# zellerlab/GECCO

Measured on AMD Instinct MI355X. Metric: genes/sec CRF decode (windowed fwd-bwd marginals + Viterbi), higher is better.
Workload: dtype f64

## Files before the change

gecco_amd/csrc/crf_vd_short.hpp:

```cpp
#pragma once

#include "crf_device.hpp"
#include "crf_scan.hpp"

namespace gecco {
namespace {

constexpr int kT = 256;
constexpr int kGPL = kSeqGenesPerLane;
constexpr int kBlockGenes = kT * kGPL;
static_assert(kBlockGenes == kSeqBlockGenes, "host tables assume this block size");

__device__ __forceinline__ double vd_max(double a, double b) {
    double r;
    asm("v_max_f64 %0, %1, %2" : "=v"(r) : "v"(a), "v"(b));
    return r;
}
__device__ __forceinline__ double vd_min(double a, double b) {
    double r;
    asm("v_min_f64 %0, %1, %2" : "=v"(r) : "v"(a), "v"(b));
    return r;
}
__device__ __forceinline__ double vd_min_abs(double a, double b) {
    double r;
    asm("v_min_f64 %0, |%1|, |%2|" : "=v"(r) : "v"(a), "v"(b));
    return r;
}
__device__ __forceinline__ double vd_max_s(double a, double bound) {
    double r;
    asm("v_max_f64 %0, %1, %2" : "=v"(r) : "v"(a), "s"(bound));
    return r;
}
__device__ __forceinline__ double vd_min_s(double a, double bound) {
    double r;
    asm("v_min_f64 %0, %1, %2" : "=v"(r) : "v"(a), "s"(bound));
    return r;
}
__device__ __forceinline__ void vd_shift_in_gt(uint32_t &acc, double x, double bound) {
    asm("v_cmp_lt_f64 vcc, %2, %1\n\tv_addc_co_u32 %0, vcc, %0, %0, vcc" : "+v"(acc) : "v"(x), "s"(bound) : "vcc");
}
struct COp {
    static __device__ __forceinline__ CE identity() { return CE{0.0, -__builtin_huge_val(), __builtin_huge_val()}; }
    static __device__ __forceinline__ CE combine(const CE &a, const CE &b) {
        return CE{a.a + b.a, vd_min(vd_max(a.L + b.a, b.L), b.H), vd_min(vd_max(a.H + b.a, b.L), b.H)};
    }
    static __device__ __forceinline__ void combine_into(CE &t, CE &v) {
        asm volatile(
            "v_add_f64 %[tl], %[tl], %[a]\n\t"
            "v_add_f64 %[th], %[th], %[a]\n\t"
            "v_add_f64 %[a], %[ta], %[a]\n\t"
            "v_max_f64 %[tl], %[tl], %[L]\n\t"
            "v_max_f64 %[th], %[th], %[L]\n\t"
            "v_min_f64 %[L], %[tl], %[H]\n\t"
            "v_min_f64 %[H], %[th], %[H]"
            : [a] "+v"(v.a), [L] "+v"(v.L), [H] "+v"(v.H), [tl] "+v"(t.L), [th] "+v"(t.H)
            : [ta] "v"(t.a));
    }
};

__device__ __forceinline__ double vd_bound(const SeqArgs &A, double nnz, double n) { return nnz * A.v_wmax2 + (n + 2.0) * A.v_tmax; }
constexpr double kVdEps = 2.220446049250313e-16;
__device__ __forceinline__ double vd_margin(double r, double ulpM) { return (4.0 * r + 4.0) * ulpM; }

constexpr int kFixChunk = 1024;
struct FixStage {
    double2 st[kFixChunk];
    uint32_t bpw[kFixChunk / 16];
};
__device__ __forceinline__ void exact_states(const SeqArgs &A, int g0, int m, FixStage &fx, int first_lane) {
    const int nl = kT - first_lane, me = int(threadIdx.x) - first_lane;
    if (me < 0) return;
    for (int base = me; base < m; base += 4 * nl) {
        int lo[4], hi[4];
        double s0[4], s1[4];
        int longest = 0;
#pragma unroll
        for (int u = 0; u < 4; ++u) {
            const int i = base + u * nl;
            lo[u] = hi[u] = 0;
            if (i < m) {
                lo[u] = A.csr_gene_ptr[g0 + i];
                hi[u] = A.csr_gene_ptr[g0 + i + 1];
            }
            s0[u] = s1[u] = 0.0;
        }
#pragma unroll
        for (int u = 0; u < 4; ++u) longest = max(longest, hi[u] - lo[u]);
        for (int k = 0; k < longest; ++k) {
            int a[4];
#pragma unroll
            for (int u = 0; u < 4; ++u) a[u] = lo[u] + k < hi[u] ? A.csr_attr_id[lo[u] + k] : -1;
            double2 w[4];
#pragma unroll
            for (int u = 0; u < 4; ++u) w[u] = unsigned(a[u]) < unsigned(A.csr_n_attrs) ? A.csr_wtab01[a[u]] : make_double2(0.0, 0.0);
#pragma unroll
            for (int u = 0; u < 4; ++u) {
                s0[u] += w[u].x;
                s1[u] += w[u].y;
            }
        }
#pragma unroll
        for (int u = 0; u < 4; ++u) {
            const int i = base + u * nl;
            if (i < m) fx.st[i] = make_double2(s0[u], s1[u]);
        }
    }
}
__device__ __forceinline__ void exact_walk(const SeqArgs &A, FixStage &fx, int m, bool first, double &d0, double &d1) {
    int i = 0;
    if (first) {
        d0 = fx.st[0].x;
        d1 = fx.st[0].y;
        i = 1;
    }
    auto step = [&](const double2 s) {
        const double a0 = d0 + A.t00, b0 = d1 + A.t10;
        const double a1 = d0 + A.t01, b1 = d1 + A.t11;
        d0 = fmax(a0, b0) + s.x;
        d1 = fmax(a1, b1) + s.y;
    };
    for (; i < m && (i & 7); ++i) {
        step(fx.st[i]);
        fx.st[i] = make_double2(d0, d1);
    }
    for (; i + 8 <= m; i += 8) {
        double2 sv[8];
#pragma unroll
        for (int u = 0; u < 8; ++u) sv[u] = fx.st[i + u];
#pragma unroll
        for (int u = 0; u < 8; ++u) {
            step(sv[u]);
            fx.st[i + u] = make_double2(d0, d1);
        }
    }
    for (; i < m; ++i) {
        step(fx.st[i]);
        fx.st[i] = make_double2(d0, d1);
    }
}
__device__ __forceinline__ void exact_backpointers(const SeqArgs &A, FixStage &fx, int m, bool first, double e0, double e1) {
    for (int w = threadIdx.x; 16 * w < m; w += kT) {
        uint32_t word = 0;
        for (int i = max(16 * w, first ? 1 : 0); i < min(16 * w + 16, m); ++i) {
            const double p0 = i ? fx.st[i - 1].x : e0, p1 = i ? fx.st[i - 1].y : e1;
            const uint32_t arg0 = (p0 + A.t00) < (p1 + A.t10) ? 1u : 0u, arg1 = (p0 + A.t01) < (p1 + A.t11) ? 1u : 0u;
            word |= (arg0 | (arg1 << 1)) << (2 * (i & 15));
        }
        fx.bpw[w] = word;
    }
}
__device__ __forceinline__ uint32_t *exact_bp_words(const SeqArgs &A, int gs) { return reinterpret_cast<uint32_t *>(A.alpha) + size_t(gs); }
__device__ __forceinline__ uint32_t *exact_end_labels(const SeqArgs &A, int gs) {
    return reinterpret_cast<uint32_t *>(A.alpha) + size_t(A.n_genes) + size_t(gs);
}
__device__ __forceinline__ void exact_backtrack(const SeqArgs &A, int gs, int ge, double d0, double d1) {
    const int n = ge - gs, nw = (n + 15) / 16;
    uint32_t *bpc = exact_bp_words(A, gs), *endl = exact_end_labels(A, gs);
    auto word_map = [&](uint32_t bits, int w, uint32_t y) {
        const int hi = min(16 * w + 15, n - 1), lo = max(16 * w, 1);
        for (int t = hi; t >= lo; --t) y = (bits >> (2 * (t & 15) + y)) & 1u;
        return y;
    };
    for (int w = threadIdx.x; w < nw; w += kT) {
        const uint32_t bits = bpc[w];
        endl[w] = word_map(bits, w, 0) | (word_map(bits, w, 1) << 1);
    }
    __syncthreads();
    if (threadIdx.x == 0) {
        uint32_t y = d0 < d1 ? 1u : 0u;
        for (int w = nw - 1; w >= 0; --w) {
            const uint32_t mp = endl[w];
            endl[w] = y;
            y = (mp >> y) & 1u;
        }
    }
    __syncthreads();
    for (int w = threadIdx.x; w < nw; w += kT) {
        const uint32_t bits = bpc[w];
        uint32_t y = endl[w];
        const int hi = min(16 * w + 15, n - 1), lo = 16 * w;
        for (int t = hi; t >= lo; --t) {
            A.y[gs + t] = int8_t(y);
            if (t >= 1) y = (bits >> (2 * (t & 15) + y)) & 1u;
        }
    }
    __syncthreads();
}

__device__ __forceinline__ void exact_delta_contig(const SeqArgs &A, int gs, int ge, FixStage &fx) {
    uint32_t *bpc = exact_bp_words(A, gs);
    double d0 = 0.0, d1 = 0.0;
    for (int cb = gs; cb < ge; cb += kFixChunk) {
        const int m = min(kFixChunk, ge - cb);
        const double e0 = d0, e1 = d1;
        exact_states(A, cb, m, fx, 0);
        __syncthreads();
        if (threadIdx.x == 0) exact_walk(A, fx, m, cb == gs, d0, d1);
        __syncthreads();
        d0 = fx.st[m - 1].x;
        d1 = fx.st[m - 1].y;
        exact_backpointers(A, fx, m, cb == gs, e0, e1);
        __syncthreads();
        for (int i = threadIdx.x; i < (m + 15) / 16; i += kT) bpc[(cb - gs) / 16 + i] = fx.bpw[i];
        __syncthreads();
    }
    exact_backtrack(A, gs, ge, d0, d1);
}

constexpr double kVdPad = 1e30;

struct VdShortSmem {
    double st[kT * (kGPL + 1)];
    uint32_t mark[kBlockGenes / 32];
    int c_end;
    CE tot[kT / 64];
    uint32_t mtot[kT / 64];
    double pv[kT / 64];
    uint32_t pbad[kT / 64];
    uint32_t vote[kT / 64];
};
static_assert(sizeof(VdShortSmem) <= 20480, "eight workgroups per CU");
__device__ __forceinline__ void load_short(const double *__restrict__ v, int g0, int n, VdShortSmem &stg, double (&x)[kGPL]) {
    const int base = int(threadIdx.x) * kGPL;
    const double *vp = v + g0;
    double *row = stg.st + threadIdx.x * (kGPL + 1);
    const int wave_end = (__builtin_amdgcn_readfirstlane(int(threadIdx.x >> 6)) + 1) * 64 * kGPL;
    if (wave_end <= n) {
#pragma unroll
        for (int k = 0; k < kGPL; ++k) x[k] = vp[base + k];
#pragma unroll
        for (int k = 0; k < kGPL; ++k) row[k] = x[k];
        return;
    }
#pragma unroll
    for (int k = 0; k < kGPL; ++k) x[k] = vp[max(min(base + k, n - 1), 0)];
#pragma unroll
    for (int k = 0; k < kGPL; ++k) {
        x[k] = base + k < n ? x[k] : kVdPad;
        row[k] = x[k];
    }
}

__device__ __forceinline__ uint32_t wave_or_u32(uint32_t v) {
    v |= uint32_t(__builtin_amdgcn_update_dpp(0, int(v), 0x111, 0xF, 0xF, true));
    v |= uint32_t(__builtin_amdgcn_update_dpp(0, int(v), 0x112, 0xF, 0xF, true));
    v |= uint32_t(__builtin_amdgcn_update_dpp(0, int(v), 0x114, 0xF, 0xF, true));
    v |= uint32_t(__builtin_amdgcn_update_dpp(0, int(v), 0x118, 0xF, 0xF, true));
    v |= uint32_t(__builtin_amdgcn_update_dpp(0, int(v), 0x142, 0xA, 0xF, true));
    v |= uint32_t(__builtin_amdgcn_update_dpp(0, int(v), 0x143, 0xC, 0xF, true));
    return uint32_t(__builtin_amdgcn_readlane(int(v), 63));
}

constexpr int kVdRun = 6;
__device__ __forceinline__ void vd_apply(const CE &P, double in, double &v) {
    asm volatile("v_add_f64 %0, %1, %2\n\tv_max_f64 %0, %0, %3\n\tv_min_f64 %0, %0, %4" : "+v"(v) : "v"(in), "v"(P.a), "v"(P.L), "v"(P.H));
}
__device__ __forceinline__ void vd_propagate(const CE &P, double &v, uint64_t &known) {
    for (int it = 0; it < kVdRun; ++it) {
        const uint64_t todo = (known << 1) & ~known;
        if (!todo) break;
        const double in = dpp_f64_z<0x138>(v);
        if (__builtin_amdgcn_inverse_ballot_w64(todo)) vd_apply(P, in, v);
        known |= todo;
    }
}

__device__ __forceinline__ void vd_short_block(const SeqArgs &A, const int blk, VdShortSmem &stg) {
    CE *lds = stg.tot;
    uint32_t *ldsm = stg.mtot;
    const int slot = threadIdx.x;
    const int g0 = __builtin_amdgcn_readfirstlane(A.cblk[blk]), n = __builtin_amdgcn_readfirstlane(A.cblk[blk + 1]) - g0;
    const uint32_t bits = A.lane_bits[blk * kT + slot];
    const uint32_t first = bits & 0xffu, last = bits >> 8;
    const uint32_t wave_bits = wave_or_u32(bits);
    double x[kGPL];
    load_short(A.dstate, g0, n, stg, x);
    const int cnt = min(kGPL, n - slot * kGPL);
    const double *row = stg.st + slot * (kGPL + 1);
    CE P = COp::identity();
#pragma unroll
    for (int k = 0; k < kGPL; ++k) {
        const double dvk = x[k];
        const bool fst = (first >> k) & 1u;
        const double c = A.v_k + dvk;
        const double l2 = vd_min_s(vd_max_s(P.L, A.v_lo), A.v_hi) + c, h2 = vd_min_s(vd_max_s(P.H, A.v_lo), A.v_hi) + c;
        P.a += c;
        P.L = l2;
        P.H = h2;
        if ((wave_bits >> k) & 1u) {
            asm volatile("" ::: "memory");
            P.L = fst ? dvk : l2;
            P.H = fst ? dvk : h2;
        }
    }
    double Din;
    {
        const int wave = __builtin_amdgcn_readfirstlane(int(threadIdx.x >> 6));
        double v = P.L;
        uint64_t known = __builtin_amdgcn_ballot_w64(P.L == P.H);
        vd_propagate(P, v, known);
        const bool wave_bad = (known | (known - 1)) != ~uint64_t(0) || !(known & (wave ? (uint64_t(2) << kVdRun) - 1 : uint64_t(1)));
        if ((threadIdx.x & 63) == 63) stg.pv[wave] = v;
        block_or_post(wave_bad, stg.pbad);
        __syncthreads();
        if (block_or_read(stg.pbad)) {
            const CE M = block_scan_exclusive<COp, false, CE, kScanThreads, true, true>(P, lds, static_cast<CE *>(nullptr));
            Din = M.L;
        } else {
            const double carry = stg.pv[wave ? wave - 1 : 0];
            if (!(known & 1u)) {
                if ((threadIdx.x & 63) == 0) vd_apply(P, carry, v);
                known |= 1u;
                vd_propagate(P, v, known);
            }
            Din = dpp_f64<0x138, 0xF>(carry, v);
        }
    }
    double ulpM = 0.0, margin = 1e-6 * fmax(1.0, fmax(fabs(A.v_lo), fabs(A.v_hi)));
    if (A.csr_gene_ptr) {
        ulpM = vd_bound(A, double(A.csr_gene_ptr[g0 + n] - A.csr_gene_ptr[g0]), double(n)) * kVdEps;
        margin = vd_margin(double(n), ulpM);
    }
    ulpM = __hiloint2double(__builtin_amdgcn_readfirstlane(__double2hiint(ulpM)), __builtin_amdgcn_readfirstlane(__double2loint(ulpM)));
    margin = __hiloint2double(__builtin_amdgcn_readfirstlane(__double2hiint(margin)), __builtin_amdgcn_readfirstlane(__double2loint(margin)));
    uint32_t maps = 0, lane_map;
    bool sensitive = false;
    {
        double Dq = Din, nearest = __builtin_huge_val();
#pragma unroll
        for (int k = 0; k < kGPL; ++k) {
            const double dvk = row[k];
            const double stepped = vd_min_s(vd_max_s(Dq, A.v_lo), A.v_hi) + (A.v_k + dvk);
            Dq = stepped;
            if ((wave_bits >> k) & 1u) {
                asm volatile("" ::: "memory");
                Dq = ((first >> k) & 1u) ? dvk : stepped;
            }
            vd_shift_in_gt(maps, Dq, A.v_lo);
            vd_shift_in_gt(maps, Dq, A.v_hi);
            double dist = vd_min_abs(Dq - A.v_hi, Dq - A.v_lo);
            if ((wave_bits >> (8 + k)) & 1u) {
                asm volatile("" ::: "memory");
                const bool lst = (last >> k) & 1u;
                maps = lst ? ((maps & ~3u) | (Dq > 0.0 ? 3u : 0u)) : maps;
                dist = lst ? fabs(Dq) : dist;
            }
            nearest = vd_min(nearest, dist);
        }
        sensitive = nearest <= margin;
    }
    auto label_map = [&]() {
        uint32_t y0 = 0u, y1 = 1u;
#pragma unroll
        for (int k = kGPL - 1; k >= 0; --k) {
            y0 = __builtin_amdgcn_ubfe(maps, uint32_t(2 * (kGPL - 1 - k)) | y0, 1u);
            y1 = __builtin_amdgcn_ubfe(maps, uint32_t(2 * (kGPL - 1 - k)) | y1, 1u);
        }
        return y0 | (y1 << 1);
    };
    const bool lane_sensitive = sensitive && A.v_exact;
    int vote = lane_sensitive ? 1 : 0;
    uint32_t mtotal;
    lane_map = label_map();
    uint32_t lab = block_scan_exclusive_back<MapOp>(lane_map, ldsm, &mtotal, &vote, stg.vote) & 1u;
    const bool wg_sensitive = vote != 0;
    if (wg_sensitive) {
        double Dq = Din;
        uint64_t sat = 0;
#pragma unroll
        for (int k = 0; k < kGPL; ++k) {
            if (k < cnt) {
                const double dvk = row[k];
            Dq = ((first >> k) & 1u) ? dvk : fmin(fmax(Dq, A.v_lo), A.v_hi) + (A.v_k + dvk);
                const uint64_t c = Dq >= A.v_hi + margin ? 1u : (Dq <= A.v_lo - margin ? 2u : 0u);
                sat |= c << (8 * k);
            }
        }
        *reinterpret_cast<uint64_t *>(&stg.st[slot * (kGPL + 1) + kGPL]) = sat;
        __syncthreads();
    } else {
        sensitive = false;
    }
    bool lane_flagged = false;
    if (sensitive && cnt > 0) {
        double D = 0.0;
        int r = 0;
        auto certain = [&](double x) { return x >= A.v_hi + margin || x <= A.v_lo - margin; };
        if (!(first & 1u)) {
            const int t0 = slot * kGPL;
            int p = t0 - 1;
            auto dval = [&](int t) { return stg.st[(t / kGPL) * (kGPL + 1) + t % kGPL]; };
            for (;; --p) {
                if (A.flags[g0 + p] & 1u) {
                    D = dval(p);
                    r = 0;
                    break;
                }
                const uint32_t c = reinterpret_cast<const uint8_t *>(&stg.st[((p - 1) / kGPL) * (kGPL + 1) + kGPL])[(p - 1) % kGPL];
                if (c) {
                    D = (c == 1u ? A.v_hi : A.v_lo) + (A.v_k + dval(p));
                    r = 1;
                    break;
                }
            }
            for (int t = p + 1; t < t0; ++t) {
                r = certain(D) ? 1 : r + 1;
                D = fmin(fmax(D, A.v_lo), A.v_hi) + (A.v_k + dval(t));
            }
        }
        maps = 0;
#pragma unroll
        for (int k = 0; k < kGPL; ++k) {
            if (k < cnt) {
                const double dvk = row[k];
                const bool fst = (first >> k) & 1u;
                r = fst ? 0 : (certain(D) ? 1 : r + 1);
                D = fst ? dvk : fmin(fmax(D, A.v_lo), A.v_hi) + (A.v_k + dvk);
                const bool lst = (last >> k) & 1u;
                const double thi = lst ? 0.0 : A.v_hi, tlo = lst ? 0.0 : A.v_lo;
                maps |= ((D > thi ? 1u : 0u) | (D > tlo ? 2u : 0u)) << (2 * (kGPL - 1 - k));
                const double mr = vd_margin(double(r), ulpM);
                lane_flagged |= fabs(D - thi) <= mr || fabs(D - tlo) <= mr;
            }
        }
        if (A.vd_stats) {
            atomicAdd(A.vd_stats + 0, 1u);
            if (lane_flagged) atomicAdd(A.vd_stats + 1, 1u);
        }
    }
    bool wg_flagged = false;
    if (wg_sensitive) {
        block_or_post(lane_flagged, stg.vote);
        __syncthreads();
        wg_flagged = block_or_read(stg.vote);
        lane_map = label_map();
        lab = block_scan_exclusive_back<MapOp>(lane_map, ldsm, &mtotal) & 1u;
    }
    uint64_t packed = 0;
#pragma unroll
    for (int k = kGPL - 1; k >= 0; --k) {
        lab = __builtin_amdgcn_ubfe(maps, uint32_t(2 * (kGPL - 1 - k)) | lab, 1u);
        packed |= uint64_t(lab) << (8 * k);
    }
    {
        struct __attribute__((packed)) Bytes8 {
            uint64_t v;
        };
        int8_t *yp = A.y + g0 + slot * kGPL;
        if (cnt >= kGPL) {
            reinterpret_cast<Bytes8 *>(yp)->v = packed;
        } else {
            for (int k = 0; k < cnt; ++k) yp[k] = int8_t(packed >> (8 * k));
        }
    }
    if (wg_flagged && A.csr_gene_ptr) {
        uint32_t *mark = stg.mark;
        int *c_end = &stg.c_end;
        __syncthreads();
        if (slot < kBlockGenes / 32) mark[slot] = 0;
        __syncthreads();
        if (lane_flagged) {
            int prev = -1;
            for (int k = 0; k < cnt; ++k) {
                int t = slot * kGPL + k;
                while (!(A.flags[g0 + t] & 1u)) --t;
                if (t != prev) atomicOr(&mark[t >> 5], 1u << (t & 31));
                prev = t;
            }
        }
        __syncthreads();
        FixStage &st2 = *reinterpret_cast<FixStage *>(stg.st);
        static_assert(sizeof(stg.st) >= sizeof(FixStage), "exact pass: LDS for one chunk of state scores");
        for (int wi = 0; wi < kBlockGenes / 32; ++wi) {
            uint32_t bits = mark[wi];
            while (bits) {
                const int cs = wi * 32 + __builtin_ctz(bits);
                bits &= bits - 1;
                if (slot == 0) *c_end = n;
                __syncthreads();
                for (int i = cs + slot; i < n; i += kT)
                    if (A.flags[g0 + i] & 2u) {
                        atomicMin(c_end, i + 1);
                        break;
                    }
                __syncthreads();
                const int ce = *c_end;
                __syncthreads();
                if (slot == 0 && A.vd_stats) {
                    atomicAdd(A.vd_stats + 2, 1u);
                    atomicAdd(A.vd_stats + 3, uint32_t(ce - cs));
                }
                exact_delta_contig(A, g0 + cs, g0 + ce, st2);
            }
        }
    }
}

}
}
```

Before: 78.29 billion.

## Replace block map scan with carry-chain bit arithmetic for Viterbi labels

New measurement: 79.15 billion (median of 6 runs). 1.01x the previous value.

```diff
diff --git a/gecco_amd/csrc/crf_vd_short.hpp b/gecco_amd/csrc/crf_vd_short.hpp
--- a/gecco_amd/csrc/crf_vd_short.hpp
+++ b/gecco_amd/csrc/crf_vd_short.hpp
@@ -214,11 +214,11 @@
     uint32_t mark[kBlockGenes / 32];
     int c_end;
     CE tot[kT / 64];
-    uint32_t mtot[kT / 64];
     double pv[kT / 64];
     uint32_t pbad[kT / 64];
-    uint32_t vote[kT / 64];
+    uint32_t chain;
 };
+static_assert(kT / 64 == 4, "one byte per wave in VdShortSmem::chain");
 static_assert(sizeof(VdShortSmem) <= 20480, "eight workgroups per CU");
 __device__ __forceinline__ void load_short(const double *__restrict__ v, int g0, int n, VdShortSmem &stg, double (&x)[kGPL]) {
     const int base = int(threadIdx.x) * kGPL;
@@ -265,9 +265,38 @@
     }
 }
 
+__device__ __forceinline__ uint32_t vd_lane_sum(uint32_t maps) { return (((maps >> 1) & 0x5555u) | 0xAAAAu) + (maps & 0x5555u); }
+__device__ __forceinline__ uint64_t vd_lane_labels(uint32_t S) {
+    const uint32_t R = __builtin_bitreverse32(~S & 0xAAAAu) >> 16;
+    const uint32_t lo4 = __umul24(R & 0xFFu, 0x41041u) & 0x01010101u, hi4 = __umul24((R >> 8) & 0xFFu, 0x41041u) & 0x01010101u;
+    return uint64_t(lo4) | (uint64_t(hi4) << 32);
+}
+struct VdChain {
+    uint64_t a, b;
+};
+__device__ __forceinline__ VdChain vd_chain_post(uint32_t maps, uint32_t S0, bool vote, uint32_t *word) {
+    const int wave = __builtin_amdgcn_readfirstlane(int(threadIdx.x >> 6));
+    const uint64_t P = __builtin_amdgcn_ballot_w64(maps == 0xAAAAu), G = __builtin_amdgcn_ballot_w64((S0 & 0x10000u) != 0u);
+    const uint64_t rest = ~P;
+    const uint32_t total = rest ? (((G >> __builtin_ctzll(rest)) & 1u) ? 3u : 0u) : 2u;
+    const uint32_t post = (__builtin_amdgcn_ballot_w64(vote) != 0 ? 1u : 0u) | (total << 1);
+    if ((threadIdx.x & 63) == 63) reinterpret_cast<uint8_t *>(word)[wave] = uint8_t(post);
+    return VdChain{__builtin_bitreverse64(G | P), __builtin_bitreverse64(G)};
+}
+__device__ __forceinline__ uint32_t vd_chain_resolve(const VdChain &c, const uint32_t *word, bool *vote) {
+    const int wave = __builtin_amdgcn_readfirstlane(int(threadIdx.x >> 6));
+    const uint32_t all = uint32_t(__builtin_amdgcn_readfirstlane(int(*word)));
+    *vote = (all & 0x01010101u) != 0u;
+    uint32_t y = 0;
+#pragma unroll
+    for (int w = kT / 64 - 1; w >= 1; --w)
+        if (w > wave) y = (all >> (8 * w + 1 + int(y))) & 1u;
+    const uint64_t s = c.a + c.b + y;
+    return __builtin_amdgcn_inverse_ballot_w64(__builtin_bitreverse64(s ^ c.a ^ c.b)) ? 1u : 0u;
+}
+
 __device__ __forceinline__ void vd_short_block(const SeqArgs &A, const int blk, VdShortSmem &stg) {
     CE *lds = stg.tot;
-    uint32_t *ldsm = stg.mtot;
     const int slot = threadIdx.x;
     const int g0 = __builtin_amdgcn_readfirstlane(A.cblk[blk]), n = __builtin_amdgcn_readfirstlane(A.cblk[blk + 1]) - g0;
     const uint32_t bits = A.lane_bits[blk * kT + slot];
@@ -323,7 +352,7 @@
     }
     ulpM = __hiloint2double(__builtin_amdgcn_readfirstlane(__double2hiint(ulpM)), __builtin_amdgcn_readfirstlane(__double2loint(ulpM)));
     margin = __hiloint2double(__builtin_amdgcn_readfirstlane(__double2hiint(margin)), __builtin_amdgcn_readfirstlane(__double2loint(margin)));
-    uint32_t maps = 0, lane_map;
+    uint32_t maps = 0;
     bool sensitive = false;
     {
         double Dq = Din, nearest = __builtin_huge_val();
@@ -349,21 +378,14 @@
         }
         sensitive = nearest <= margin;
     }
-    auto label_map = [&]() {
-        uint32_t y0 = 0u, y1 = 1u;
-#pragma unroll
-        for (int k = kGPL - 1; k >= 0; --k) {
-            y0 = __builtin_amdgcn_ubfe(maps, uint32_t(2 * (kGPL - 1 - k)) | y0, 1u);
-            y1 = __builtin_amdgcn_ubfe(maps, uint32_t(2 * (kGPL - 1 - k)) | y1, 1u);
-        }
-        return y0 | (y1 << 1);
-    };
-    const bool lane_sensitive = sensitive && A.v_exact;
-    int vote = lane_sensitive ? 1 : 0;
-    uint32_t mtotal;
-    lane_map = label_map();
-    uint32_t lab = block_scan_exclusive_back<MapOp>(lane_map, ldsm, &mtotal, &vote, stg.vote) & 1u;
-    const bool wg_sensitive = vote != 0;
+    bool wg_sensitive;
+    uint32_t S0 = vd_lane_sum(maps);
+    uint32_t lab;
+    {
+        const VdChain chain = vd_chain_post(maps, S0, sensitive && A.v_exact, &stg.chain);
+        __syncthreads();
+        lab = vd_chain_resolve(chain, &stg.chain, &wg_sensitive);
+    }
     if (wg_sensitive) {
         double Dq = Din;
         uint64_t sat = 0;
@@ -430,18 +452,12 @@
     }
     bool wg_flagged = false;
     if (wg_sensitive) {
-        block_or_post(lane_flagged, stg.vote);
-        __syncthreads();
-        wg_flagged = block_or_read(stg.vote);
-        lane_map = label_map();
-        lab = block_scan_exclusive_back<MapOp>(lane_map, ldsm, &mtotal) & 1u;
-    }
-    uint64_t packed = 0;
-#pragma unroll
-    for (int k = kGPL - 1; k >= 0; --k) {
-        lab = __builtin_amdgcn_ubfe(maps, uint32_t(2 * (kGPL - 1 - k)) | lab, 1u);
-        packed |= uint64_t(lab) << (8 * k);
-    }
+        S0 = vd_lane_sum(maps);
+        const VdChain chain = vd_chain_post(maps, S0, lane_flagged, &stg.chain);
+        __syncthreads();
+        lab = vd_chain_resolve(chain, &stg.chain, &wg_flagged);
+    }
+    const uint64_t packed = vd_lane_labels(S0 + lab);
     {
         struct __attribute__((packed)) Bytes8 {
             uint64_t v;
```
